# MIT-SPARK/Khronos

Hardware: NVIDIA H100
Metric: rgbd_frames_per_sec_integrated (higher is better)
Workload: dtype f32

## Files before the change

### khronos_b200/csrc/kb_api.cu

```cuda
#include <algorithm>
#include <climits>
#include <cmath>
#include <cstdio>
#include <cstdlib>
#include <cstring>
#include <string>
#include <thread>
#include <type_traits>
#include <vector>

#include "../../include/khronos_b200.h"
#include "kb_kernels.cuh"
#include "kb_mesh.cuh"
#include "kb_motion_device.cuh"
#include "kb_objects_device.cuh"
#include "kb_tracks_device.cuh"
#include "kb_motion_host.h"

using namespace kb;

struct kb_handle {
  kb_map_config map{};
  kb_integrator_config integ{};
  kb_tracking_config trk{};
// ... 1025 lines not shown
      v.label = f.label ? h->stg_label + off : nullptr;
      v.mask = f.mask ? h->stg_mask + off : nullptr;
      v.object_image = f.object_image ? h->stg_object + off : nullptr;
      v.depth16 = f.depth_u16 ? h->stg_depth16 + off : nullptr;
      v.label8 = (f.label_u8 || narrowed[b]) ? h->stg_label8 + off : nullptr;
    }
    v.depth_scale = f.depth_u16_scale;
    if (v.depth16) v.depth = h->stg_depth + off;
    if (v.label8) v.label = h->stg_label + off;
    if (!v.depth) return fail(h, KB_ERR_INVALID, "frame without depth image");
    if (f.mask == KB_MASK_LAST_DETECTION)
      v.mask = h->motion_have_image ? h->d_dynamic : nullptr;
    v.tiles = h->tile_max + tile_set + static_cast<size_t>(b) * h->tile_stride;
    if (allocate_blocks) {
      const float reach = c.max_range + p.infl;
      const float inv = 1.f / h->block_size;
      for (int a = 0; a < 3; ++a) {
        lo[a] = std::min(lo[a], static_cast<int>(std::floor((tw[a] - reach) * inv)));
        hi[a] = std::max(hi[a], static_cast<int>(std::floor((tw[a] + reach) * inv)));
      }
    }
  }
  if (any_host) {
    auto copyKind = [&](auto member, auto* staging, size_t per = 1) -> int {
      using T = std::remove_pointer_t<decltype(staging)>;
      const size_t img = px * per;
      int b = 0;
      while (b < n) {
        const T* src = (frames[b].memory == KB_MEM_DEVICE) ? nullptr : static_cast<const T*>(frames[b].*member);
        if (!src || static_cast<const void*>(src) == static_cast<const void*>(KB_MASK_LAST_DETECTION)) { ++b; continue; }
        int e = b + 1;
        while (e < n && frames[e].memory != KB_MEM_DEVICE && static_cast<const T*>(frames[e].*member) == src + static_cast<size_t>(e - b) * img) ++e;
        T* dst = staging + (static_cast<size_t>(set) * kMaxBatch + b) * img;
        KB_CUDA(h, cudaMemcpyAsync(dst, src, static_cast<size_t>(e - b) * img * sizeof(T), cudaMemcpyHostToDevice, h->copy_stream));
        b = e;
      }
      return KB_OK;
    };
    int cst;
    if ((cst = copyKind(&kb_frame::depth, h->stg_depth)) != KB_OK) return cst;
    if (!any_narrowed) {
      if ((cst = copyKind(&kb_frame::label, h->stg_label)) != KB_OK) return cst;
    } else {
      for (int b = 0; b < n;) {
        if (narrowed[b]) {
          int e = b + 1;
          while (e < n && narrowed[e]) ++e;
          const size_t o = (static_cast<size_t>(set) * kMaxBatch + b) * px;
          KB_CUDA(h, cudaMemcpyAsync(h->stg_label8 + o, h->pin_label8 + o, static_cast<size_t>(e - b) * px, cudaMemcpyHostToDevice, h->copy_stream));
          b = e;
        } else {
          if (frames[b].memory != KB_MEM_DEVICE && frames[b].label) {
            const size_t o = (static_cast<size_t>(set) * kMaxBatch + b) * px;
            KB_CUDA(h, cudaMemcpyAsync(h->stg_label + o, frames[b].label, px * sizeof(int32_t), cudaMemcpyHostToDevice, h->copy_stream));
          }
          ++b;
        }
      }
    }
    if ((cst = copyKind(&kb_frame::mask, h->stg_mask)) != KB_OK) return cst;
    if ((cst = copyKind(&kb_frame::object_image, h->stg_object)) != KB_OK) return cst;
    if ((cst = copyKind(&kb_frame::depth_u16, h->stg_depth16)) != KB_OK) return cst;
    if ((cst = copyKind(&kb_frame::label_u8, h->stg_label8)) != KB_OK) return cst;
    if (any_host_color && (cst = copyKind(&kb_frame::color, h->stg_color, 3)) != KB_OK) return cst;
    KB_CUDA(h, cudaEventRecord(h->stg_ready[set], h->copy_stream));
    KB_CUDA(h, cudaStreamWaitEvent(h->stream, h->stg_ready[set], 0));
  }
  if (allocate_blocks) {
    for (int a = 0; a < 3; ++a) { p.lo[a] = lo[a]; p.dims[a] = hi[a] - lo[a] + 1; }
    h->hwm_dirty = true;
  } else {
    if (h->hwm_dirty) {
      int st, nslots = 0;
      if ((st = slotHwm(h, &nslots)) != KB_OK) return st;
      h->hwm_cached = nslots;
      h->hwm_dirty = false;
    }
    p.n_slots = h->hwm_cached;
  }
  any_compact = any_compact || any_narrowed;
  bool all_compact = any_compact;
  for (int b = 0; b < n; ++b) all_compact = all_compact && frames[b].depth_u16 != nullptr && frames[b].label == nullptr;
  p.compact_taps = all_compact ? 1 : 0;
  cudaStream_t ps = h->stream;
  if (pipe) {
    ps = h->pre_stream;
    if (any_host) KB_CUDA(h, cudaStreamWaitEvent(ps, h->stg_ready[set], 0));
    KB_CUDA(h, cudaStreamWaitEvent(ps, h->fuse_done[par], 0));
    if (h->main_dirty) {
      KB_CUDA(h, cudaEventRecord(h->main_front, h->stream));
      KB_CUDA(h, cudaStreamWaitEvent(ps, h->main_front, 0));
      h->main_dirty = false;
    }
    KB_CUDA(h, cudaMemsetAsync(h->dm.counters + kCtrWork0 + par, 0, sizeof(int), ps));
    KB_CUDA(h, cudaMemsetAsync(h->dm.counters + p.fetch_ctr, 0, sizeof(int), ps));
  }
  if (!pipe && h->pipelined) {
    KB_CUDA(h, cudaMemsetAsync(h->dm.counters + kCtrWork0 + par, 0, sizeof(int), ps));
  }
  if (any_compact && !all_compact) launchExpandFrames(p, ps);
  if (p.cull) launchTileMax(p, ps);
  launchSelectBlocks(h->dm, p, h->cull_grid, ps);
  if (pipe) {
    KB_CUDA(h, cudaEventRecord(h->pre_done[par], ps));
    KB_CUDA(h, cudaStreamWaitEvent(h->stream, h->pre_done[par], 0));
  }
  launchFuse(h->dm, p, h->fuse_grid, h->stream);
  if (pipe) KB_CUDA(h, cudaEventRecord(h->fuse_done[par], h->stream));
  KB_CUDA(h, cudaGetLastError());
  if (use_staging) KB_CUDA(h, cudaEventRecord(h->stg_consumed[set], h->stream));
  if (any_host) {
    bool must_wait = false;
    for (int b = 0; b < n; ++b) must_wait |= frames[b].memory == KB_MEM_HOST;
    if (must_wait) KB_CUDA(h, cudaStreamSynchronize(h->copy_stream));
  }
  h->ctr_dirty = true;
  return KB_OK;
}

int kb_integrate_frames(kb_handle* h, const kb_frame* frames, int32_t n_frames, int allocate_blocks,
                        kb_frame_stats* stats) {
  if (!h || !frames || n_frames < 0) return fail(h, KB_ERR_INVALID, "null frames");
  if (!h->has_cam) return fail(h, KB_ERR_STATE, "kb_set_camera must be called first");
  for (int i = 0; i < n_frames; ++i) {
    if (!frames[i].depth && !frames[i].depth_u16) return fail(h, KB_ERR_INVALID, "frame without depth image");
    for (int k = 0; k < 16; ++k)
      if (!std::isfinite(frames[i].world_T_sensor[k])) return fail(h, KB_ERR_INVALID, "non-finite sensor pose");
  }
  KB_CUDA(h, cudaSetDevice(h->device));
  int st;
  if (stats && h->ctr_dirty) {
    if ((st = readCounters(h)) != KB_OK) return st;
    std::memcpy(h->prev_ctr, h->h_ctr, sizeof(h->prev_ctr));
    h->ctr_dirty = false;
  }
  if (!h->own_stream) h->main_dirty = true;
  for (int i = 0; i < n_frames; i += kMaxBatch) {
    if ((st = integrateBatch(h, frames + i, std::min(kMaxBatch, n_frames - i), allocate_blocks)) != KB_OK) return st;
  }
  if (stats) {
    if ((st = readCounters(h)) != KB_OK) return st;
    const int* c1 = h->h_ctr;
    const int* c0 = h->prev_ctr;
    auto d = [&](int k) { return static_cast<int32_t>(static_cast<uint32_t>(c1[k]) - static_cast<uint32_t>(c0[k])); };
    stats->blocks_in_frustum = d(kCtrFrustum);
    stats->blocks_allocated = d(kCtrAllocated);
    stats->blocks_updated = d(kCtrBlocksUpdated);
    stats->voxels_updated = d(kCtrVoxelsUpdated);
    stats->voxels_in_band = d(kCtrVoxelsBand);
    stats->voxels_semantic = d(kCtrVoxelsSemantic);
    stats->total_blocks = c1[kCtrLiveBlocks];
    stats->capacity_exceeded = c1[kCtrCapacityExceeded];
    std::memcpy(h->prev_ctr, h->h_ctr, sizeof(h->prev_ctr));
    h->ctr_dirty = false;
    if (c1[kCtrCapacityExceeded]) return fail(h, KB_ERR_CAPACITY, "block / semantic pool exhausted");
  }
  return KB_OK;
}

int kb_integrate_frame(kb_handle* h, const kb_frame* f, int allocate_blocks, kb_frame_stats* stats) {
  return kb_integrate_frames(h, f, f ? 1 : 0, allocate_blocks, stats);
}

int kb_get_totals(kb_handle* h, kb_frame_stats* t) {
  if (!h || !t) return KB_ERR_INVALID;
  KB_CUDA(h, cudaSetDevice(h->device));
// ... 1195 lines not shown
```

### khronos_b200/csrc/kb_kernels.cu

```cuda
#include <limits.h>

#include <algorithm>

#include "../../include/khronos_b200.h"
#include "kb_kernels.cuh"

namespace kb {

namespace {

constexpr int kThreads = 256;
constexpr int kFuseThreads = 128;
#ifndef KB_FUSE_MIN_BLOCKS
#define KB_FUSE_MIN_BLOCKS 10
#endif
#ifndef KB_FUSE_COLOR_MIN_BLOCKS
#define KB_FUSE_COLOR_MIN_BLOCKS 8
#endif

__device__ __forceinline__ void xform(const float* R, const float* t, float x, float y, float z,
                                      float& ox, float& oy, float& oz) {
  ox = ((R[0] * x + R[1] * y) + R[2] * z) + t[0];
  oy = ((R[3] * x + R[4] * y) + R[5] * z) + t[1];
  oz = ((R[6] * x + R[7] * y) + R[8] * z) + t[2];
}

__device__ __forceinline__ bool inFrustum(const BatchParams& p, float x, float y, float z) {
  const float infl = p.infl;
  if (z < -infl) return false;
  const float r = sqrtf((x * x + y * y) + z * z);
  if (r < p.min_range - infl || r > p.max_range + infl) return false;
  if (p.pl[0][0] * x + p.pl[0][1] * z < -infl) return false;
  if (p.pl[1][0] * x + p.pl[1][1] * z < -infl) return false;
  if (p.pl[2][0] * y + p.pl[2][1] * z < -infl) return false;
  if (p.pl[3][0] * y + p.pl[3][1] * z < -infl) return false;
  return true;
}

template <bool COMPACT>
__device__ __forceinline__ float depthAt(const FrameView& f, int i) {
  if (COMPACT) return static_cast<float>(__ldg(&f.depth16[i])) * f.depth_scale;
  return __ldg(&f.depth[i]);
}
template <bool COMPACT>
__device__ __forceinline__ int labelAt(const FrameView& f, int i) {
  if (COMPACT) return static_cast<int>(__ldg(&f.label8[i]));
  return __ldg(&f.label[i]);
}

struct Taps {
  bool valid, bilinear;
  int u, v;
  float w0, w1, w2, w3;
};

template <bool COMPACT>
__device__ __forceinline__ Taps nearestTaps(const BatchParams& p, const FrameView& f, float u, float v) {
  Taps t;
  t.bilinear = false;
  t.u = static_cast<int>(roundf(u));
  t.v = static_cast<int>(roundf(v));
  t.w0 = t.w1 = t.w2 = t.w3 = 0.f;
  t.valid = t.u >= 0 && t.u < p.W && t.v >= 0 && t.v < p.H && depthAt<COMPACT>(f, t.v * p.W + t.u) > 0.f;
  return t;
}

template <bool COMPACT>
__device__ __forceinline__ Taps computeTaps(const BatchParams& p, const FrameView& f, float u, float v, float& range) {
  Taps t;
  t.valid = false;
  if (p.interp == KB_INTERP_NEAREST) {
    t = nearestTaps<COMPACT>(p, f, u, v);
    if (t.valid) range = depthAt<COMPACT>(f, t.v * p.W + t.u);
    return t;
  }
  const int u0 = static_cast<int>(floorf(u)), v0 = static_cast<int>(floorf(v));
  const bool inside = u0 >= 0 && v0 >= 0 && u0 + 1 < p.W && v0 + 1 < p.H;
  bool use_nearest = !inside;
  float r0 = 0.f, r1 = 0.f, r2 = 0.f, r3 = 0.f;
  if (inside) {
    const int i0 = v0 * p.W + u0;
    r0 = depthAt<COMPACT>(f, i0);
    r2 = depthAt<COMPACT>(f, i0 + 1);
    r1 = depthAt<COMPACT>(f, i0 + p.W);
    r3 = depthAt<COMPACT>(f, i0 + p.W + 1);
    const bool all_valid = r0 > 0.f && r1 > 0.f && r2 > 0.f && r3 > 0.f;
    if (p.interp == KB_INTERP_ADAPTIVE) {
      const float mx = fmaxf(fmaxf(r0, r1), fmaxf(r2, r3));
      const float mn = fminf(fminf(r0, r1), fminf(r2, r3));
      use_nearest = !all_valid || !(mx - mn < p.adaptive_thr);
    } else if (!all_valid) {
      return t;
    }
  } else if (p.interp != KB_INTERP_ADAPTIVE) {
    return t;
// ... 298 lines not shown
  i = __shfl_sync(0xffffffffu, i, 0);
  if (i < p.max_work && lane < p.items_per_block) p.item_fmask[static_cast<size_t>(i) * p.items_per_block + lane] = p.cull ? 0u : mask;
}

constexpr int kCullChunk = 1;
template <int VPS>
__global__ void __launch_bounds__(128) itemCullKernel(const DeviceMap m, const __grid_constant__ BatchParams p) {
  constexpr int ITEMS = (VPS / 4) * (VPS / 8) * (VPS / 4);
  const int lane = threadIdx.x & 31;
  const int warp = (blockIdx.x * blockDim.x + threadIdx.x) >> 5;
  const int n_warps = (gridDim.x * blockDim.x) >> 5;
  const int chunks = (p.n_frames + kCullChunk - 1) / kCullChunk;
  const int n = min(m.counters[kCtrWork0 + p.parity], p.max_work) * chunks;
  for (int w = warp; w < n; w += n_warps) {
    const int wi = w / chunks, ch = w % chunks;
    const uint32_t bmask = p.work_masks[wi] & (((kCullChunk >= 32 ? 0u : (1u << kCullChunk)) - 1u) << (ch * kCullChunk));
    if (!bmask || lane >= ITEMS) continue;
    const int3 bi = m.block_index[p.work_slots[wi]];
    int x0, y0, z0;
    itemOrigin<VPS>(lane, x0, y0, z0);
    const float ox = static_cast<float>(bi.x) * p.block_size, oy = static_cast<float>(bi.y) * p.block_size,
                oz = static_cast<float>(bi.z) * p.block_size;
    const float lx = ox + (static_cast<float>(x0) + 0.5f) * p.voxel_size, hx = ox + (static_cast<float>(x0 + 3) + 0.5f) * p.voxel_size;
    const float ly = oy + (static_cast<float>(y0) + 0.5f) * p.voxel_size, hy = oy + (static_cast<float>(y0 + 7) + 0.5f) * p.voxel_size;
    const float lz = oz + (static_cast<float>(z0) + 0.5f) * p.voxel_size, hz = oz + (static_cast<float>(z0 + 3) + 0.5f) * p.voxel_size;
    uint32_t keep = 0, rem = bmask;
    while (rem) {
      const int b = __ffs(rem) - 1;
      rem &= rem - 1;
      if (!boxCulledLane(p, p.f[b], lx, ly, lz, hx, hy, hz)) keep |= 1u << b;
    }
    if (keep) atomicOr(&p.item_fmask[static_cast<size_t>(wi) * ITEMS + lane], keep);
  }
}

template <int VPS, bool PB>
__global__ void __launch_bounds__(256) itemCompactKernel(const DeviceMap m, const __grid_constant__ BatchParams p) {
  constexpr int kItems = PB ? kCtrItemsB0 : kCtrItems0;
  constexpr int BOXES = (VPS / 4) * (VPS / 8) * (VPS / 4);
  const int n = min(m.counters[kCtrWork0 + p.parity], p.max_work) * BOXES;
  const int lane = threadIdx.x & 31;
  for (int base = (blockIdx.x * blockDim.x + threadIdx.x) - lane; base < n; base += gridDim.x * blockDim.x) {
    const int i = base + lane;
    const uint32_t fm = i < n ? p.item_fmask[i] : 0u;
    const int cls = fm ? (32 - __popc(fm)) >> 2 : -1;
    const unsigned peers = __match_any_sync(0xffffffffu, cls);
    if (cls < 0) continue;
    const int leader = __ffs(peers) - 1;
    int start = 0;
    if (lane == leader) start = atomicAdd(&m.counters[kItems + cls], __popc(peers));
    start = __shfl_sync(peers, start, leader);
    const int idx = start + __popc(peers & ((1u << lane) - 1u));
    if (idx < p.item_list_cap) p.item_list[static_cast<size_t>(cls) * p.item_list_cap + idx] = i;
  }
}

template <bool PB>
__device__ __forceinline__ int listedBox(const BatchParams& p, const int (&n_cls)[kItemClasses], int j) {
  int k = 0;
#pragma unroll
  for (int c = 0; c < kItemClasses - 1; ++c) {
    if (k == c && j >= n_cls[c]) { j -= n_cls[c]; k = c + 1; }
  }
  return p.item_list[static_cast<size_t>(k) * p.item_list_cap + j];
}

__device__ __noinline__ uint32_t trackingFold(const DeviceMap& m, const TrackEval& t, uint32_t born, size_t gi) {
  const uint8_t fl = m.vflags[gi];
  const uint32_t c_stored = m.last_occ[gi];
  uint32_t c_true;
  bool act, rem;
  evalTracking(m, t, born, m.last_obs[gi], c_stored, fl, &c_true, &act, &rem);
  if (c_true != c_stored) m.last_occ[gi] = c_true;
  return (fl & kVoxEverFree) | (act ? kVoxActive : 0) | (rem ? kVoxToRemove : 0);
}

template <int VPS, int LPI, bool COMPACT, bool COLOR, bool LIST = false, bool PB = false>
__global__ void __launch_bounds__(kFuseThreads, COLOR ? KB_FUSE_COLOR_MIN_BLOCKS : KB_FUSE_MIN_BLOCKS) fuseKernel(const __grid_constant__ DeviceMap m, const __grid_constant__ BatchParams p) {
  constexpr int kFetch = PB ? kCtrFetchB : kCtrFetch;
  [[maybe_unused]] constexpr int kItems = PB ? kCtrItemsB0 : kCtrItems0;
  constexpr int V = VPS * VPS * VPS;
  constexpr int NK = 4;
  constexpr int BOXES = (VPS / 4) * (VPS / 8) * (VPS / NK);
  extern __shared__ float s_rows[];
  const int lane = threadIdx.x & 31;
  constexpr int lpi = LPI, ipb = NK / LPI;
  int n_cls[kItemClasses] = {0};
  int n_items;
  if constexpr (LIST) {
    n_items = 0;
#pragma unroll
    for (int c = 0; c < kItemClasses; ++c) {
      n_cls[c] = min(m.counters[kItems + c], p.item_list_cap);
      n_items += n_cls[c];
    }
    n_items *= ipb;
  } else {
    n_items = min(m.counters[kCtrWork0 + p.parity], p.max_work) * BOXES * ipb;
  }
  const bool binary = p.sem_mode == KB_SEMANTICS_BINARY;
  const int L = p.L;
  int n_valid = 0, n_band = 0, n_sem = 0;

  int pending = 0;
  if (lane == 0) pending = atomicAdd(&m.counters[kFetch], 1);
  for (;;) {
    const int w = __shfl_sync(0xffffffffu, pending, 0);
    if (w >= n_items) break;
    if (lane == 0) pending = atomicAdd(&m.counters[kFetch], 1);
    int box = w / ipb;
    if constexpr (LIST) {
      box = listedBox<PB>(p, n_cls, box);
    }
    const uint32_t fmask = p.item_fmask[box];
    if (!fmask) continue;
    const int wi = box / BOXES, it = box % BOXES;
    const int slot = p.work_slots[wi];
    const int3 bi = m.block_index[slot];
    const int sem = L > 0 ? m.block_sem[slot] : -1;
    int x0, y0, z0;
    itemOrigin<VPS>(it, x0, y0, z0);
    uint32_t upd_all = 0;
    bool any_have = false;
#pragma unroll 1
    for (int k = (w % ipb) * lpi; k < (w % ipb) * lpi + lpi; ++k) {
    const int vx = x0 + (lane & 3), vy = y0 + (lane >> 2), vz = z0 + k;
    const int lin = vx + VPS * (vy + VPS * vz);
    const size_t gi = static_cast<size_t>(slot) * V + lin;
    const float wx = static_cast<float>(bi.x) * p.block_size + (static_cast<float>(vx) + 0.5f) * p.voxel_size;
    const float wy = static_cast<float>(bi.y) * p.block_size + (static_cast<float>(vy) + 0.5f) * p.voxel_size;
    const float wz = static_cast<float>(bi.z) * p.block_size + (static_cast<float>(vz) + 0.5f) * p.voxel_size;
    float2 st = make_float2(0.f, 0.f);
    uint32_t lobs = 0, vfl = 0, upd_frames = 0;
    bool have = false, row_resident = false;
    int best_label = 0;
    uchar4 col = make_uchar4(0, 0, 0, 0);
    bool col_dirty = false;

    uint32_t rem = fmask;
    while (rem) {
      const int b = __ffs(rem) - 1;
      rem &= rem - 1;
      const FrameView& f = p.f[b];
      const bool has_label_img = L > 0 && (binary ? f.object_image != nullptr : (COMPACT ? f.label8 != nullptr : f.label != nullptr));
      float x, y, z;
      xform(f.R, f.t, wx, wy, wz, x, y, z);
      if (z <= 0.f) continue;
      const float u = p.fx * x / z + p.cx;
      const float v = p.fy * y / z + p.cy;
      if (u < 0.f || u > static_cast<float>(p.W - 1) || v < 0.f || v > static_cast<float>(p.H - 1)) continue;
      float range = 0.f;
      const Taps taps = computeTaps<COMPACT>(p, f, u, v, range);
      if (!taps.valid) continue;
      const float sdf = range - z;
      if (sdf < -p.trunc) continue;
      const bool in_band = fabsf(sdf) < p.trunc;
      uint32_t label = 0;
      if (in_band) {
        const int ti = tapIndex(p, taps);
        if (f.mask != nullptr && __ldg(&f.mask[ti]) != 0) continue;
        if (has_label_img) {
          if (binary) {
            label = __ldg(&f.object_image[ti]) == f.target_id ? 1u : 0u;
          } else {
            label = static_cast<uint32_t>(labelAt<COMPACT>(f, ti));
            if (label < static_cast<uint32_t>(KB_MAX_LABELS) && ((p.blocked_mask >> label) & 1ull)) continue;
          }
        }
      }
      const float wm = measurementWeight(p, z, sdf);
      if (!have) {
        st = m.tsdf[gi];
        have = true;
        if (p.with_tracking) vfl = trackingFold(m, p.trk, m.born_frame[slot], gi);
        if constexpr (COLOR) col = m.color[gi];
      }
      const float sdf_c = fminf(fmaxf(sdf, -p.trunc), p.trunc);
      const float2 old = st;
      st.x = (old.x * old.y + sdf_c * wm) / (old.y + wm);
      st.y = fminf(old.y + wm, p.max_weight);
      lobs = f.frame_idx;
      upd_frames |= 1u << b;
      ++n_valid;
      if (!in_band) continue;
      ++n_band;
      if constexpr (COLOR) {
        if (f.color != nullptr) {
          const uchar3 cm = measuredColor(p, f, taps);
          const float tot = old.y + wm;
          const float ratio = tot > 0.f ? wm / tot : 0.f;
          col.x = mergeChannel(col.x, cm.x, ratio);
          col.y = mergeChannel(col.y, cm.y, ratio);
          col.z = mergeChannel(col.z, cm.z, ratio);
          col_dirty = true;
        }
      }
      if (sem >= 0 && has_label_img && label < static_cast<uint32_t>(L)) {
        const size_t si = static_cast<size_t>(sem) * V + lin;
        if (!row_resident) {
          row_resident = true;
          const bool empty = m.sem_label[si] == kSemEmpty;
          if (binary) {
            const float2 c = empty ? make_float2(0.f, 0.f) : *reinterpret_cast<const float2*>(m.sem_lik + si * 2);
            s_rows[threadIdx.x] = c.x;
            s_rows[kFuseThreads + threadIdx.x] = c.y;
          } else {
            const float4* __restrict__ lk = reinterpret_cast<const float4*>(m.sem_lik + si * m.Lp);
            for (int k4 = 0; k4 < m.Lp; k4 += 4) {
              const float4 c = empty ? make_float4(p.mle_init, p.mle_init, p.mle_init, p.mle_init) : lk[k4 >> 2];
              s_rows[(k4 + 0) * kFuseThreads + threadIdx.x] = c.x;
              s_rows[(k4 + 1) * kFuseThreads + threadIdx.x] = c.y;
              s_rows[(k4 + 2) * kFuseThreads + threadIdx.x] = c.z;
              s_rows[(k4 + 3) * kFuseThreads + threadIdx.x] = c.w;
            }
          }
        }
        if (binary) {
          const float c = s_rows[label * kFuseThreads + threadIdx.x] + 1.f;
          s_rows[label * kFuseThreads + threadIdx.x] = c;
          best_label = s_rows[kFuseThreads + threadIdx.x] > s_rows[threadIdx.x] ? 1 : 0;
        } else {
          for (int k2 = 0; k2 < m.Lp; k2 += 2) {
            float c0 = s_rows[(k2 + 0) * kFuseThreads + threadIdx.x], c1 = s_rows[(k2 + 1) * kFuseThreads + threadIdx.x];
            c0 += static_cast<uint32_t>(k2 + 0) == label ? p.mle_diag : p.mle_off;
            c1 += static_cast<uint32_t>(k2 + 1) == label ? p.mle_diag : p.mle_off;
            s_rows[(k2 + 0) * kFuseThreads + threadIdx.x] = c0;
            s_rows[(k2 + 1) * kFuseThreads + threadIdx.x] = c1;
          }
        }
        ++n_sem;
      }
    }

    if (have) {
      m.tsdf[gi] = st;
      if constexpr (COLOR) {
        if (col_dirty) m.color[gi] = col;
      }
      if (p.with_tracking) {
        m.last_obs[gi] = lobs;
        m.vflags[gi] = static_cast<uint8_t>(vfl | (st.x < p.occ_thr ? 0 : kVoxNotOccupied));
      }
      if (row_resident) {
        const size_t si = static_cast<size_t>(sem) * V + lin;
        if (binary) {
          *reinterpret_cast<float2*>(m.sem_lik + si * 2) = make_float2(s_rows[threadIdx.x], s_rows[kFuseThreads + threadIdx.x]);
        } else {
          float4* __restrict__ lk = reinterpret_cast<float4*>(m.sem_lik + si * m.Lp);
          for (int k4 = 0; k4 < m.Lp; k4 += 4)
            lk[k4 >> 2] = make_float4(s_rows[(k4 + 0) * kFuseThreads + threadIdx.x], s_rows[(k4 + 1) * kFuseThreads + threadIdx.x],
                                      s_rows[(k4 + 2) * kFuseThreads + threadIdx.x], s_rows[(k4 + 3) * kFuseThreads + threadIdx.x]);
        }
        if (!binary) {
          float bestv = s_rows[threadIdx.x];
          best_label = 0;
          for (int kk = 1; kk < L; ++kk) {
            const float c = s_rows[kk * kFuseThreads + threadIdx.x];
            if (c > bestv) { bestv = c; best_label = kk; }
          }
        }
        m.sem_label[si] = static_cast<uint16_t>(best_label);
      }
    }
    upd_all |= upd_frames;
    any_have |= have;
    }
    if (__any_sync(0xffffffffu, any_have)) {
      uint32_t upd_frames = upd_all;
#pragma unroll
      for (int o = 16; o > 0; o >>= 1) upd_frames |= __shfl_xor_sync(0xffffffffu, upd_frames, o);
      if (lane == 0) {
        const uint32_t all = KB_FLAG_UPDATED | KB_FLAG_MESH_UPDATED | KB_FLAG_ESDF_UPDATED | KB_FLAG_TRACKING_UPDATED;
        if ((m.block_flags[slot] & all) != all) atomicOr(&m.block_flags[slot], all);
        if ((p.work_upd[wi] & upd_frames) != upd_frames) {
          const uint32_t prev = atomicOr(&p.work_upd[wi], upd_frames);
          const int fresh = __popc(upd_frames & ~prev);
          if (fresh) {
            atomicAdd(&m.counters[kCtrBlocksUpdated], fresh);
            atomicAdd(&totals64(m.counters)[kTotBlocksUpdated], static_cast<unsigned long long>(fresh));
          }
        }
      }
    }
  }
  n_valid = warpSum(n_valid);
  if (n_valid) {
    n_band = warpSum(n_band);
    n_sem = warpSum(n_sem);
    if (lane == 0) {
      unsigned long long* t64 = totals64(m.counters);
      atomicAdd(&m.counters[kCtrVoxelsUpdated], n_valid);
      atomicAdd(&t64[kTotVoxelsUpdated], static_cast<unsigned long long>(n_valid));
      if (n_band) {
        atomicAdd(&m.counters[kCtrVoxelsBand], n_band);
        atomicAdd(&t64[kTotVoxelsBand], static_cast<unsigned long long>(n_band));
      }
      if (n_sem) {
        atomicAdd(&m.counters[kCtrVoxelsSemantic], n_sem);
        atomicAdd(&t64[kTotVoxelsSemantic], static_cast<unsigned long long>(n_sem));
      }
    }
  }
}

template <int VPS, bool COMPACT, bool PB>
__global__ void __launch_bounds__(kFuseThreads, KB_FUSE_MIN_BLOCKS) fuseKernelCoop(const __grid_constant__ DeviceMap m, const __grid_constant__ BatchParams p) {
  constexpr int kFetch = PB ? kCtrFetchB : kCtrFetch;
  constexpr int kItems = PB ? kCtrItemsB0 : kCtrItems0;
  constexpr int V = VPS * VPS * VPS;
  constexpr int NK = 4;
  constexpr int BOXES = (VPS / 4) * (VPS / 8) * (VPS / NK);
  constexpr uint8_t kInvalid = 0xFE, kNoSem = 0xFF;
  extern __shared__ float s_dyn[];
  const int rows_floats = max(m.Lp, 2) * 32;
  float* __restrict__ s_rows = s_dyn;
  float* __restrict__ s_w = s_dyn + rows_floats;
  float* __restrict__ s_s = s_w + 32 * 32;
  uint8_t* __restrict__ s_l = reinterpret_cast<uint8_t*>(s_s + 32 * 32);
  __shared__ int s_item;
  const int warp = threadIdx.x >> 5, lane = threadIdx.x & 31;
  int n_cls[kItemClasses];
  int n_items = 0;
#pragma unroll
  for (int c = 0; c < kItemClasses; ++c) {
    n_cls[c] = min(m.counters[kItems + c], p.item_list_cap);
    n_items += n_cls[c];
  }
  n_items *= NK;
  const bool binary = p.sem_mode == KB_SEMANTICS_BINARY;
  const int L = p.L;
  int n_valid = 0, n_band = 0, n_sem = 0;
  int pending = 0;
  if (threadIdx.x == 0) pending = atomicAdd(&m.counters[kFetch], 1);
  for (;;) {
    if (threadIdx.x == 0) s_item = pending;
    __syncthreads();
    const int w = s_item;
    if (w >= n_items) break;
    if (threadIdx.x == 0) pending = atomicAdd(&m.counters[kFetch], 1);
    const int box = listedBox<PB>(p, n_cls, w / NK);
    const uint32_t fmask = p.item_fmask[box];
// ... 1016 lines not shown
  for (int lin = threadIdx.x; lin < V; lin += blockDim.x) {
    const size_t src = static_cast<size_t>(slot) * V + lin, dst = static_cast<size_t>(blockIdx.x) * V + lin;
    const uint8_t f = m.vflags[src];
    const uint32_t o = m.last_obs[src];
    uint32_t c;
    bool act, rem;
    evalTracking(m, ev, born, o, m.last_occ[src], f, &c, &act, &rem);
    last_obs[dst] = stamps[o];
    last_occ[dst] = stamps[c];
    ever_free[dst] = (f & kVoxEverFree) ? 1 : 0;
    active[dst] = act ? 1 : 0;
    to_remove[dst] = rem ? 1 : 0;
    any_active |= act ? 1 : 0;
  }
  any_active = __syncthreads_or(any_active);
  if (threadIdx.x == 0) {
    const bool seen = ev.k_last != 0 && ev.k_last >= born;
    block_active[blockIdx.x] = (seen && any_active && !(m.block_flags[slot] & kFlagInactiveOverride)) ? 1 : 0;
  }
}

__global__ void gatherColorKernel(const DeviceMap m, const int* slots, uint8_t* rgb) {
  const int V = m.V, slot = slots[blockIdx.x];
  for (int lin = threadIdx.x; lin < V; lin += blockDim.x) {
    const uchar4 c = m.color[static_cast<size_t>(slot) * V + lin];
    uint8_t* o = rgb + (static_cast<size_t>(blockIdx.x) * V + lin) * 3;
    o[0] = c.x; o[1] = c.y; o[2] = c.z;
  }
}

__global__ void gatherSemanticKernel(const DeviceMap m, const int* slots, int L, uint32_t* label,
                                     uint8_t* empty, float* lik) {
  const int V = m.V, slot = slots[blockIdx.x];
  const int sem = m.block_sem[slot];
  for (int lin = threadIdx.x; lin < V; lin += blockDim.x) {
    const size_t dst = static_cast<size_t>(blockIdx.x) * V + lin;
    uint16_t lb = kSemEmpty;
    if (sem >= 0) lb = m.sem_label[static_cast<size_t>(sem) * V + lin];
    const bool is_empty = lb == kSemEmpty;
    label[dst] = is_empty ? 0u : lb;
    empty[dst] = is_empty ? 1 : 0;
    if (lik) {
      for (int k = 0; k < L; ++k)
        lik[dst * L + k] = is_empty ? 0.f : m.sem_lik[(static_cast<size_t>(sem) * V + lin) * m.Lp + k];
    }
  }
}

}

void launchExpandFrames(const BatchParams& p, cudaStream_t s) {
  expandFramesKernel<<<dim3(smCount(), p.n_frames), 256, 0, s>>>(p);
}
void launchExpandDepth(const uint16_t* src, float scale, float* dst, int n, cudaStream_t s) {
  expandDepthKernel<<<(n + 255) / 256, 256, 0, s>>>(src, scale, dst, n);
}
void launchTileMax(const BatchParams& p, cudaStream_t s) {
  bool vec4 = !p.compact_taps && (p.W % 4) == 0;
  for (int b = 0; b < p.n_frames && vec4; ++b) vec4 = (reinterpret_cast<uintptr_t>(p.f[b].depth) & 15u) == 0;
  if (vec4) {
    const int warps = ((p.W + 127) / 128) * p.lvl_ty[1];
    tileMaxVec4Kernel<<<dim3((warps + 7) / 8, p.n_frames), 256, 0, s>>>(p);
  } else {
    const int warps = ((p.W + 31) / 32) * p.lvl_ty[1];
    tileMaxKernel<<<dim3((warps + 7) / 8, p.n_frames), 256, 0, s>>>(p);
  }
  tilePyramidKernel<<<p.n_frames, 256, 0, s>>>(p);
}
void launchSelectBlocks(const DeviceMap& m, const BatchParams& p, int cull_grid, cudaStream_t s) {
  const int n = p.allocate ? p.dims[0] * p.dims[1] * p.dims[2] : p.n_slots;
  if (p.pipelined) selectBlocksKernel<true><<<(std::max(n, 1) + 3) / 4, 128, 0, s>>>(m, p);
  else selectBlocksKernel<false><<<(std::max(n, 1) + 3) / 4, 128, 0, s>>>(m, p);
  if (p.cull) {
    if (m.vps == 16) itemCullKernel<16><<<cull_grid, 128, 0, s>>>(m, p);
    else itemCullKernel<8><<<cull_grid, 128, 0, s>>>(m, p);
  }
  if (p.item_list) {
    const bool pb = p.fetch_ctr == kCtrFetchB;
    cudaMemsetAsync(m.counters + (pb ? kCtrItemsB0 : kCtrItems0), 0, kItemClasses * sizeof(int), s);
    if (m.vps == 16) { if (pb) itemCompactKernel<16, true><<<cull_grid, 256, 0, s>>>(m, p); else itemCompactKernel<16, false><<<cull_grid, 256, 0, s>>>(m, p); }
    else { if (pb) itemCompactKernel<8, true><<<cull_grid, 256, 0, s>>>(m, p); else itemCompactKernel<8, false><<<cull_grid, 256, 0, s>>>(m, p); }
  }
}
static size_t fuseSmemBytes(int Lp) { return static_cast<size_t>(std::max(Lp, 2)) * kFuseThreads * sizeof(float); }
int fuseBlocksPerSm(int vps, int Lp) {
  int n = 0;
  if (vps == 16) cudaOccupancyMaxActiveBlocksPerMultiprocessor(&n, fuseKernel<16, 1, false, false>, kFuseThreads, fuseSmemBytes(Lp));
  else cudaOccupancyMaxActiveBlocksPerMultiprocessor(&n, fuseKernel<8, 1, false, false>, kFuseThreads, fuseSmemBytes(Lp));
  return n > 0 ? n : 4;
}
void launchFuse(const DeviceMap& m, const BatchParams& p, int grid, cudaStream_t s) {
  if (grid <= 0) return;
  const size_t smem = fuseSmemBytes(m.Lp);
  const bool one = p.layers_per_item == 1, c = p.compact_taps != 0, col = p.has_color != 0 && m.color != nullptr;
  const bool pb = p.fetch_ctr == kCtrFetchB;
#define KB_FUSE(V, LP, C)                                                                        \
  do {                                                                                           \
    if (pb) {                                                                                    \
      if (col) fuseKernel<V, LP, C, true, false, true><<<grid, kFuseThreads, smem, s>>>(m, p);   \
      else if (p.item_list) fuseKernel<V, LP, C, false, true, true><<<grid, kFuseThreads, smem, s>>>(m, p); \
      else fuseKernel<V, LP, C, false, false, true><<<grid, kFuseThreads, smem, s>>>(m, p);      \
    } else {                                                                                     \
      if (col) fuseKernel<V, LP, C, true><<<grid, kFuseThreads, smem, s>>>(m, p);                \
      else if (p.item_list) fuseKernel<V, LP, C, false, true><<<grid, kFuseThreads, smem, s>>>(m, p); \
      else fuseKernel<V, LP, C, false><<<grid, kFuseThreads, smem, s>>>(m, p);                   \
    }                                                                                            \
  } while (0)
#define KB_FUSE_MLP_G(V, LP, C, GG)                                                                                  \
  do {                                                                                                               \
    if (pb) {                                                                                                        \
      if (p.item_list) fuseKernelMlp<V, LP, C, GG, true, true><<<grid, kFuseThreads, smem, s>>>(m, p);               \
      else fuseKernelMlp<V, LP, C, GG, false, true><<<grid, kFuseThreads, smem, s>>>(m, p);                          \
    } else {                                                                                                         \
      if (p.item_list) fuseKernelMlp<V, LP, C, GG, true><<<grid, kFuseThreads, smem, s>>>(m, p);                     \
      else fuseKernelMlp<V, LP, C, GG, false><<<grid, kFuseThreads, smem, s>>>(m, p);                                \
    }                                                                                                                \
  } while (0)
#define KB_FUSE_MLP(V, LP, C)                                                                                        \
  do {                                                                                                               \
    if (p.mlp_group == 2) KB_FUSE_MLP_G(V, LP, C, 2);                                                                \
    else KB_FUSE_MLP_G(V, LP, C, 4);                                                                                 \
  } while (0)
  if (p.coop && p.item_list && one && !col && p.mlp_group == 0) {
    const size_t csmem = static_cast<size_t>(std::max(m.Lp, 2)) * 32 * sizeof(float) + 2 * 32 * 32 * sizeof(float) + 32 * 32;
#define KB_COOP(V, C)                                                                   \
  do {                                                                                  \
    if (pb) fuseKernelCoop<V, C, true><<<grid, kFuseThreads, csmem, s>>>(m, p);         \
    else fuseKernelCoop<V, C, false><<<grid, kFuseThreads, csmem, s>>>(m, p);           \
  } while (0)
    if (m.vps == 16) { if (c) KB_COOP(16, true); else KB_COOP(16, false); }
    else { if (c) KB_COOP(8, true); else KB_COOP(8, false); }
#undef KB_COOP
    return;
  }
  if (p.mlp_group != 0 && !col) {
    if (m.vps == 16) {
      if (one) { if (c) KB_FUSE_MLP(16, 1, true); else KB_FUSE_MLP(16, 1, false); }
      else { if (c) KB_FUSE_MLP(16, 4, true); else KB_FUSE_MLP(16, 4, false); }
    } else {
      if (one) { if (c) KB_FUSE_MLP(8, 1, true); else KB_FUSE_MLP(8, 1, false); }
      else { if (c) KB_FUSE_MLP(8, 4, true); else KB_FUSE_MLP(8, 4, false); }
    }
    return;
  }
  if (m.vps == 16) {
    if (one) { if (c) KB_FUSE(16, 1, true); else KB_FUSE(16, 1, false); }
    else { if (c) KB_FUSE(16, 4, true); else KB_FUSE(16, 4, false); }
  } else {
    if (one) { if (c) KB_FUSE(8, 1, true); else KB_FUSE(8, 1, false); }
    else { if (c) KB_FUSE(8, 4, true); else KB_FUSE(8, 4, false); }
  }
#undef KB_FUSE
#undef KB_FUSE_MLP
#undef KB_FUSE_MLP_G
}
void launchTrackingPass(const DeviceMap& m, const TrackingParams& p, int everfree_grid, cudaStream_t s) {
  trackingPassKernel<<<(std::max(p.n_slots, 1) + 255) / 256, 256, 0, s>>>(m, p);
  if (p.everfree_v2) everFreeKernelV2<false><<<everfree_grid, kThreads, 0, s>>>(m, p);
  else everFreeKernel<false><<<everfree_grid, kThreads, 0, s>>>(m, p);
  resetPendingKernel<<<1, 1, 0, s>>>(m);
}
void launchTrackingBegin(const DeviceMap& m, const TrackingParams& p, const ShardExchange& x, int32_t* pending_out, cudaStream_t s) {
  trackingPassKernel<<<(std::max(p.n_slots, 1) + 255) / 256, 256, 0, s>>>(m, p);
  exportPendingKernel<<<(x.cap_pending + 255) / 256, 256, 0, s>>>(m, p.pending, pending_out, x.cap_pending);
}
void launchHaloPack(const DeviceMap& m, const TrackingParams& p, const ShardExchange& x, const int32_t* all_pending,
                    int32_t* halo_out, cudaStream_t s) {
// ... 130 lines not shown
```

### khronos_b200/csrc/kb_kernels.cuh

```cuda
#pragma once

#include "kb_device.cuh"

namespace kb {

constexpr int kTileLevels = 4;
constexpr int kMaxBatch = 32;

struct FrameView {
  float R[9], t[3];
  const float* depth;
  const int* label;
  const int* mask;
  const int* object_image;
  const uint8_t* color;
  float* tiles;
  const uint16_t* depth16;
  const uint8_t* label8;
  float depth_scale;
  uint32_t frame_idx;
  int target_id;
};

struct BatchParams {
  int W, H;
  float fx, fy, cx, cy, min_range, max_range;
  float pl[4][2];
  float voxel_size, block_size, trunc, infl;
  int use_dropoff;
  float dropoff_eps;
  int constant_weight;
  float max_weight;
  int interp;
  float adaptive_thr;
  int sem_mode, L;
  float mle_diag, mle_off, mle_init;
  unsigned long long blocked_mask;
  int lo[3], dims[3];
  int allocate;
  int n_slots;
  int rank, nranks;
  int with_tracking;
  TrackEval trk;
  float occ_thr;
  int n_frames;
  int parity;
  int compact_taps;
  int cull;
  int has_color;
  int lvl_tx[kTileLevels], lvl_ty[kTileLevels], lvl_off[kTileLevels];
  int* work_slots;
  uint32_t* work_masks;
  uint32_t* work_upd;
  uint32_t* item_fmask;
  int pipelined;
  int fetch_ctr;
  int items_ctr;
  int coop;
  int mlp_group;
  int* item_list;
  int item_list_cap;
  int items_per_block;
  int layers_per_item;
  int max_work;
  FrameView f[kMaxBatch];
};

struct TrackingParams {
  TrackEval ev;
  uint32_t prev_pass;
  int connectivity;
  int n_slots;
  int* pending;
  int everfree_v2;
  int rank, nranks;
  const int32_t* ghost_bits;
  const unsigned long long* ghost_keys;
  const int* ghost_vals;
  uint32_t ghost_mask;
};

constexpr int kMaxPeers = 16;
struct PeerBuffers {
  void* p[kMaxPeers];
  int n;
};

struct ShardExchange {
  int rank, nranks;
  int cap_pending, cap_halo;
  int mask_words;
  int* halo_mark;
  int* publish;
  unsigned long long* ghost_keys;
  int* ghost_vals;
  uint32_t ghost_mask;
  __host__ __device__ int pending_stride() const { return 4 + 3 * cap_pending; }
  __host__ __device__ int halo_entry() const { return 4 + mask_words; }
  __host__ __device__ int halo_stride() const { return 4 + cap_halo * halo_entry(); }
};

struct MotionParams {
  float Rw[9], tw[3];
  int W, H;
  float fx, fy, cx, cy;
  float max_range, min_z_world;
  float block_size, block_size_inv, voxel_size_inv;
  const float* depth;
  const float* vertex;
  int3* pixel_gidx;
  uint8_t* pixel_seed;
  uint8_t* pixel_flags;
};

void launchTileMax(const BatchParams& p, cudaStream_t s);
void launchExpandFrames(const BatchParams& p, cudaStream_t s);
void launchExpandDepth(const uint16_t* src, float scale, float* dst, int n, cudaStream_t s);
void launchSelectBlocks(const DeviceMap& m, const BatchParams& p, int cull_grid, cudaStream_t s);
void launchFuse(const DeviceMap& m, const BatchParams& p, int grid, cudaStream_t s);
// ... 36 lines not shown
```

Baseline: 134,200.

## Use per-thread row-major semantic smem rows with float4 access and frame bitmasks

Changes the shared-memory scratch for per-voxel label likelihoods from label-major (strided by thread count) to a per-thread row layout padded to an odd multiple of four floats, so each thread reads and writes its row with float4 operations. The MLE update becomes a vectorized add of the off-diagonal term plus a scalar fix-up of the observed label, and the write-back is fused with the argmax. Per-frame label-image and mask presence is precomputed on the host as bitmasks, which avoids pointer loads inside the per-frame loop. The padded stride slightly increases shared memory use, which may reduce occupancy, and float4 row access needs the odd-quad padding to limit bank conflicts.

After: 146,700, median of 6. 1.09x the previous value.

```diff
diff --git a/khronos_b200/csrc/kb_api.cu b/khronos_b200/csrc/kb_api.cu
--- a/khronos_b200/csrc/kb_api.cu
+++ b/khronos_b200/csrc/kb_api.cu
@@ -1131,6 +1131,16 @@
   bool all_compact = any_compact;
   for (int b = 0; b < n; ++b) all_compact = all_compact && frames[b].depth_u16 != nullptr && frames[b].label == nullptr;
   p.compact_taps = all_compact ? 1 : 0;
+  p.label_frames = 0;
+  p.mask_frames = 0;
+  for (int b = 0; b < n; ++b) {
+    const FrameView& v = p.f[b];
+    const void* lab = p.sem_mode == KB_SEMANTICS_BINARY ? static_cast<const void*>(v.object_image)
+                      : all_compact                     ? static_cast<const void*>(v.label8)
+                                                        : static_cast<const void*>(v.label);
+    if (p.L > 0 && lab != nullptr) p.label_frames |= 1u << b;
+    if (v.mask != nullptr) p.mask_frames |= 1u << b;
+  }
   cudaStream_t ps = h->stream;
   if (pipe) {
     ps = h->pre_stream;
diff --git a/khronos_b200/csrc/kb_kernels.cu b/khronos_b200/csrc/kb_kernels.cu
--- a/khronos_b200/csrc/kb_kernels.cu
+++ b/khronos_b200/csrc/kb_kernels.cu
@@ -11,6 +11,7 @@
 
 constexpr int kThreads = 256;
 constexpr int kFuseThreads = 128;
+__host__ __device__ constexpr int fuseRowStride(int Lp) { return Lp <= 2 ? 2 : ((Lp >> 2) | 1) << 2; }
 #ifndef KB_FUSE_MIN_BLOCKS
 #define KB_FUSE_MIN_BLOCKS 10
 #endif
@@ -475,7 +476,8 @@
   constexpr int V = VPS * VPS * VPS;
   constexpr int NK = 4;
   constexpr int BOXES = (VPS / 4) * (VPS / 8) * (VPS / NK);
-  extern __shared__ float s_rows[];
+  extern __shared__ float4 s_rows4[];
+  float* const s_rows = reinterpret_cast<float*>(s_rows4);
   const int lane = threadIdx.x & 31;
   constexpr int lpi = LPI, ipb = NK / LPI;
   int n_cls[kItemClasses] = {0};
@@ -535,7 +537,7 @@
       const int b = __ffs(rem) - 1;
       rem &= rem - 1;
       const FrameView& f = p.f[b];
-      const bool has_label_img = L > 0 && (binary ? f.object_image != nullptr : (COMPACT ? f.label8 != nullptr : f.label != nullptr));
+      const bool has_label_img = (p.label_frames >> b) & 1u;
       float x, y, z;
       xform(f.R, f.t, wx, wy, wz, x, y, z);
       if (z <= 0.f) continue;
@@ -551,7 +553,7 @@
       uint32_t label = 0;
       if (in_band) {
         const int ti = tapIndex(p, taps);
-        if (f.mask != nullptr && __ldg(&f.mask[ti]) != 0) continue;
+        if (((p.mask_frames >> b) & 1u) && __ldg(&f.mask[ti]) != 0) continue;
         if (has_label_img) {
           if (binary) {
             label = __ldg(&f.object_image[ti]) == f.target_id ? 1u : 0u;
@@ -599,12 +601,12 @@
             s_rows[kFuseThreads + threadIdx.x] = c.y;
           } else {
             const float4* __restrict__ lk = reinterpret_cast<const float4*>(m.sem_lik + si * m.Lp);
-            for (int k4 = 0; k4 < m.Lp; k4 += 4) {
-              const float4 c = empty ? make_float4(p.mle_init, p.mle_init, p.mle_init, p.mle_init) : lk[k4 >> 2];
-              s_rows[(k4 + 0) * kFuseThreads + threadIdx.x] = c.x;
-              s_rows[(k4 + 1) * kFuseThreads + threadIdx.x] = c.y;
-              s_rows[(k4 + 2) * kFuseThreads + threadIdx.x] = c.z;
-              s_rows[(k4 + 3) * kFuseThreads + threadIdx.x] = c.w;
+            float4* const row = s_rows4 + threadIdx.x * (fuseRowStride(m.Lp) >> 2);
+            const float4 init = make_float4(p.mle_init, p.mle_init, p.mle_init, p.mle_init);
+#pragma unroll
+            for (int q = 0; q < KB_MAX_LABELS / 4; ++q) {
+              if (4 * q >= m.Lp) break;
+              row[q] = empty ? init : lk[q];
             }
           }
         }
@@ -613,13 +615,21 @@
           s_rows[label * kFuseThreads + threadIdx.x] = c;
           best_label = s_rows[kFuseThreads + threadIdx.x] > s_rows[threadIdx.x] ? 1 : 0;
         } else {
-          for (int k2 = 0; k2 < m.Lp; k2 += 2) {
-            float c0 = s_rows[(k2 + 0) * kFuseThreads + threadIdx.x], c1 = s_rows[(k2 + 1) * kFuseThreads + threadIdx.x];
-            c0 += static_cast<uint32_t>(k2 + 0) == label ? p.mle_diag : p.mle_off;
-            c1 += static_cast<uint32_t>(k2 + 1) == label ? p.mle_diag : p.mle_off;
-            s_rows[(k2 + 0) * kFuseThreads + threadIdx.x] = c0;
-            s_rows[(k2 + 1) * kFuseThreads + threadIdx.x] = c1;
-          }
+          float* const row = s_rows + threadIdx.x * fuseRowStride(m.Lp);
+          float4* const row4 = reinterpret_cast<float4*>(row);
+          const float c_label = row[label];
+          const float off = p.mle_off;
+#pragma unroll
+          for (int q = 0; q < KB_MAX_LABELS / 4; ++q) {
+            if (4 * q >= m.Lp) break;
+            float4 c = row4[q];
+            c.x += off;
+            c.y += off;
+            c.z += off;
+            c.w += off;
+            row4[q] = c;
+          }
+          row[label] = c_label + p.mle_diag;
         }
         ++n_sem;
       }
@@ -640,16 +650,19 @@
           *reinterpret_cast<float2*>(m.sem_lik + si * 2) = make_float2(s_rows[threadIdx.x], s_rows[kFuseThreads + threadIdx.x]);
         } else {
           float4* __restrict__ lk = reinterpret_cast<float4*>(m.sem_lik + si * m.Lp);
-          for (int k4 = 0; k4 < m.Lp; k4 += 4)
-            lk[k4 >> 2] = make_float4(s_rows[(k4 + 0) * kFuseThreads + threadIdx.x], s_rows[(k4 + 1) * kFuseThreads + threadIdx.x],
-                                      s_rows[(k4 + 2) * kFuseThreads + threadIdx.x], s_rows[(k4 + 3) * kFuseThreads + threadIdx.x]);
-        }
-        if (!binary) {
-          float bestv = s_rows[threadIdx.x];
+          const float4* const row = s_rows4 + threadIdx.x * (fuseRowStride(m.Lp) >> 2);
+          float bestv = 0.f;
           best_label = 0;
-          for (int kk = 1; kk < L; ++kk) {
-            const float c = s_rows[kk * kFuseThreads + threadIdx.x];
-            if (c > bestv) { bestv = c; best_label = kk; }
+#pragma unroll
+          for (int q = 0; q < KB_MAX_LABELS / 4; ++q) {
+            if (4 * q >= m.Lp) break;
+            const float4 c = row[q];
+            lk[q] = c;
+            if (q == 0) bestv = c.x;
+            else if (4 * q < L && c.x > bestv) { bestv = c.x; best_label = 4 * q; }
+            if (4 * q + 1 < L && c.y > bestv) { bestv = c.y; best_label = 4 * q + 1; }
+            if (4 * q + 2 < L && c.z > bestv) { bestv = c.z; best_label = 4 * q + 2; }
+            if (4 * q + 3 < L && c.w > bestv) { bestv = c.w; best_label = 4 * q + 3; }
           }
         }
         m.sem_label[si] = static_cast<uint16_t>(best_label);
@@ -1832,7 +1845,7 @@
     else { if (pb) itemCompactKernel<8, true><<<cull_grid, 256, 0, s>>>(m, p); else itemCompactKernel<8, false><<<cull_grid, 256, 0, s>>>(m, p); }
   }
 }
-static size_t fuseSmemBytes(int Lp) { return static_cast<size_t>(std::max(Lp, 2)) * kFuseThreads * sizeof(float); }
+static size_t fuseSmemBytes(int Lp) { return static_cast<size_t>(fuseRowStride(Lp)) * kFuseThreads * sizeof(float); }
 int fuseBlocksPerSm(int vps, int Lp) {
   int n = 0;
   if (vps == 16) cudaOccupancyMaxActiveBlocksPerMultiprocessor(&n, fuseKernel<16, 1, false, false>, kFuseThreads, fuseSmemBytes(Lp));
diff --git a/khronos_b200/csrc/kb_kernels.cuh b/khronos_b200/csrc/kb_kernels.cuh
--- a/khronos_b200/csrc/kb_kernels.cuh
+++ b/khronos_b200/csrc/kb_kernels.cuh
@@ -35,6 +35,8 @@
   float adaptive_thr;
   int sem_mode, L;
   float mle_diag, mle_off, mle_init;
+  uint32_t label_frames;
+  uint32_t mask_frames;
   unsigned long long blocked_mask;
   int lo[3], dims[3];
   int allocate;
```
